# lior1990/hp-vae-gan

Measured on AMD Instinct MI355X. Metric: train iters/sec per pyramid scale, air_balloons 13f@144p, higher is better.
Workload: dtype f32

## Files before the change

hp-vae-gan_amd/csrc/conv_mfma.hip:

```cpp
#include "hpvg_common.h"
#include "hpvg.h"
#include <stdlib.h>

namespace {

__device__ const float g_zero_word[16] = {0.f, 0.f, 0.f, 0.f, 0.f, 0.f, 0.f, 0.f, 0.f, 0.f, 0.f, 0.f, 0.f, 0.f, 0.f, 0.f};
constexpr long HPVG_ZERO_PLANE_FLOATS = 1L << 18;
__device__ float g_zero_plane[HPVG_ZERO_PLANE_FLOATS];

#ifdef HPVG_TRACE
__device__ unsigned long long g_trace[8192 * 4];
__device__ unsigned long long g_phase[8192 * 4];
#define HPVG_PH(i) { unsigned long long now_ = __builtin_readcyclecounter(); ph_a[i] += now_ - ph_t; ph_t = now_; }
#define HPVG_PH_INIT unsigned long long ph_t = __builtin_readcyclecounter(); unsigned long long ph_a[4] = {0, 0, 0, 0};
#define HPVG_PH_END if (threadIdx.x == 0) { for (int i_ = 0; i_ < 4; ++i_) g_phase[4 * blockIdx.x + i_] = ph_a[i_]; }
#define HPVG_TRACE_BEGIN unsigned long long tr_t0 = wall_clock64(); unsigned long long tr_c0 = __builtin_readcyclecounter();
#define HPVG_TRACE_END                                                              \
  if (threadIdx.x == 0 && blockIdx.x + gridDim.x * (blockIdx.y + gridDim.y * blockIdx.z) < 8192) { \
    unsigned long long* tr = g_trace + 4 * (blockIdx.x + gridDim.x * (blockIdx.y + gridDim.y * blockIdx.z)); \
    tr[0] = tr_t0;                                                                  \
    tr[1] = wall_clock64();                                                         \
    tr[2] = __builtin_amdgcn_s_getreg((31 << 11) | 4);                              \
    tr[3] = (__builtin_amdgcn_s_getreg((31 << 11) | 20) & 0xF) | ((__builtin_readcyclecounter() - tr_c0) << 8); \
  }
// ... 161 lines not shown
#if HPVG_CONV_ASM_STAGE
        const unsigned dst_lds = (unsigned)(size_t)(lptr_t)dst;
#pragma unroll
        for (int j = 0; j < NJMAX; ++j)
          if (sl.em[j] != 0ull) conv_dma_piece(src, sl.bofs[j], dst_lds + j * 1024, sl.em[j]);
#else
#pragma unroll
        for (int j = 0; j < NJMAX; ++j)
          if ((sl.okmask >> j) & 1u)
            __builtin_amdgcn_global_load_lds((gptr_t)(src + sl.bofs[j]), (lptr_t)(dst + j * 256), 4, 0, 0);
#endif
        if (first_chunk) {
#pragma unroll
          for (int j = 0; j < NJMAX; ++j)
            if (((sl.wmask & ~sl.okmask) >> j) & 1u) xs[pl * PL + j * 256 + tid] = 0.f;
        }
      } else if (first_chunk || cg >= a.Cin) {
#pragma unroll
        for (int j = 0; j < NJMAX; ++j)
          if ((sl.wmask >> j) & 1u) xs[pl * PL + j * 256 + tid] = 0.f;
      }
    }
  } else {
#pragma unroll 2
    for (int c = 0; c < CC; ++c) {
      const int cg = ch * CC + c;
      const bool cok = cg < a.Cin;
      float sc = 1.f, sh = 0.f;
      if (cok) {
        sc = a.in_scale[cg];
        sh = a.in_shift[cg];
      }
      float v[KT][NJMAX];
#pragma unroll
      for (int dt = 0; dt < KT; ++dt) {
        const int tt = t + dt - (KT == 3 ? 1 : 0);
        const bool tok = cok && tt >= 0 && tt < a.T;
        const float* src = a.x + (((long)b * a.Cin + (cok ? cg : 0)) * a.T + (tok ? tt : 0)) * HW;
#pragma unroll
        for (int j = 0; j < NJMAX; ++j) {
          const bool ld = tok && ((sl.okmask >> j) & 1u);
          v[dt][j] = ld ? src[sl.gofs[j]] : 0.f;
        }
      }
#pragma unroll
      for (int dt = 0; dt < KT; ++dt) {
        const int tt = t + dt - (KT == 3 ? 1 : 0);
        const bool tok = cok && tt >= 0 && tt < a.T;
#pragma unroll
        for (int j = 0; j < NJMAX; ++j) {
          if ((sl.wmask >> j) & 1u) {
            float val = v[dt][j];
            if (tok && ((sl.okmask >> j) & 1u)) {
              val = val * sc + sh;
              if (a.in_lrelu) val = hpvg_lrelu(val);
            }
            xs[(c * KT + dt) * PL + j * 256 + tid] = val;
          }
        }
      }
    }
  }
}

#ifdef HPVG_CONV_WGS4
#define HPVG_CONV_WGS(MB, NB) ((MB) * (NB) <= 4 ? 4 : 2)
#else
#define HPVG_CONV_WGS(MB, NB) 2
#endif

constexpr int VAR_PLAIN = 0, VAR_MASK = 1, VAR_PRO = 2, VAR_BITS = 3;

template <int CC, int KT, int MB, int NB, int VAR>
__global__ __launch_bounds__(256, HPVG_CONV_WGS(MB, NB)) void conv_mfma_kernel(const ConvFwdArgs a) {
  constexpr int CP = CC / 2;
  constexpr int TAPS = KT * 9;
  typedef typename AVecT<CP>::type AVec;
  extern __shared__ __attribute__((aligned(16))) float xs[];

  const int tid = threadIdx.x;
  const int lane = tid & 63;
  const int wave = __builtin_amdgcn_readfirstlane(tid >> 6);
  const int half = lane >> 5, l31 = lane & 31;
  const long HW = (long)a.H * a.W;
  const int RS = a.RS, PL = a.PL;
  const float* xl = xs + half * KT * PL + l31 + wave * 32;

  HPVG_TRACE_BEGIN
  const int S = gridDim.x;
  const int g = hpvg_xcd_remap(blockIdx.x, S);
  const long Isk = (long)(a.ntl - a.skbase) * a.nchunk;
  int it = (int)((long)g * Isk / S);
  const int it_hi = (int)((long)(g + 1) * Isk / S);
  const int first_sk_tile = a.skbase + it / a.nchunk;

  HPVG_PH_INIT
  bool first_stage = true;
  for (int k = 0;; ++k) {
    int tile, ch_lo, ch_hi;
    if (k < a.ndp) {
      tile = k * S + g;
      ch_lo = 0;
      ch_hi = a.nchunk;
    } else {
      if (it >= it_hi) break;
      const int tr = it / a.nchunk;
      tile = a.skbase + tr;
      ch_lo = it - tr * a.nchunk;
      const int n = (a.nchunk - ch_lo < it_hi - it) ? a.nchunk - ch_lo : it_hi - it;
      ch_hi = ch_lo + n;
      it += n;
    }
    const SkTile tc = sk_decode_tile(a, tile, MB);
    const int b = tc.b, t = tc.t, q0 = tc.q0, w0 = tc.w0, mb0 = tc.mb0;

    const StageSlots sl = conv_stage_slots(a, q0, w0, tid);

    f32x16 acc[MB][NB];
#pragma unroll
    for (int m = 0; m < MB; ++m)
#pragma unroll
      for (int i = 0; i < NB; ++i)
#pragma unroll
        for (int e = 0; e < 16; ++e) acc[m][i][e] = 0.f;

    for (int ch = ch_lo; ch < ch_hi; ++ch) {
      if (!first_stage) __syncthreads();
      first_stage = false;
      HPVG_PH(3)
      __builtin_amdgcn_s_waitcnt(0x0F70);
      conv_stage_chunk<CC, KT, VAR == VAR_PRO>(a, xs, sl, ch, ch == ch_lo, b, t, tid, wave);
      HPVG_PH(0)
      __builtin_amdgcn_s_waitcnt(0x0F70);
      __syncthreads();
      HPVG_PH(1)

      const AVec* wpt = reinterpret_cast<const AVec*>(a.wp) + ((long)(ch * TAPS) * a.mbtot + mb0) * 64 + lane;
      AVec av[MB];
#pragma unroll
      for (int m = 0; m < MB; ++m) av[m] = wpt[m * 64];
      float bv[2][NB];
#pragma unroll
      for (int i = 0; i < NB; ++i) bv[0][i] = xl[i * 128];
#pragma unroll 1
      for (int dt = 0; dt < KT; ++dt) {
#pragma unroll
        for (int dh = 0; dh < 3; ++dh) {
#pragma unroll
          for (int dw = 0; dw < 3; ++dw) {
            wpt += (long)a.mbtot * 64;
            AVec an[MB];
#pragma unroll
            for (int m = 0; m < MB; ++m) an[m] = wpt[m * 64];
            const float* xt = xl + dt * PL + dh * RS + dw;
            const float* xn = (dw < 2) ? xt + 1 : (dh < 2 ? xl + dt * PL + (dh + 1) * RS : xl + (dt + 1 < KT ? dt + 1 : 0) * PL);
#pragma unroll
            for (int cp = 0; cp < CP; ++cp) {
              const float* nx = (cp + 1 < CP) ? xt + (2 * (cp + 1) * KT) * PL : xn;
#pragma unroll
              for (int i = 0; i < NB; ++i) bv[(cp + 1) & 1][i] = nx[i * 128];
              __builtin_amdgcn_sched_barrier(0);
              __builtin_amdgcn_s_setprio(1);
#pragma unroll
              for (int i = 0; i < NB; ++i)
#pragma unroll
                for (int m = 0; m < MB; ++m)
                  acc[m][i] = __builtin_amdgcn_mfma_f32_32x32x2f32(av[m][cp], bv[cp & 1][i], acc[m][i], 0, 0, 0);
              __builtin_amdgcn_s_setprio(0);
            }
#pragma unroll
            for (int m = 0; m < MB; ++m) av[m] = an[m];
          }
        }
      }
      HPVG_PH(2)
    }

    if (ch_lo != 0 || ch_hi != a.nchunk) {
      const int seg = (tile == first_sk_tile) ? 0 : 1;
      float* dst = a.skpart + ((long)(g * 2 + seg) * (MB * NB * 16)) * 256 + tid;
#pragma unroll
      for (int m = 0; m < MB; ++m)
#pragma unroll
        for (int i = 0; i < NB; ++i)
#pragma unroll
          for (int e = 0; e < 16; ++e) dst[((m * NB + i) * 16 + e) * 256] = acc[m][i][e];
      continue;
    }
    float bias_r[MB][16];
#pragma unroll
    for (int m = 0; m < MB; ++m)
#pragma unroll
      for (int e = 0; e < 16; ++e) {
        const int co = (mb0 + m) * 32 + (e & 3) + 8 * (e >> 2) + 4 * half;
        bias_r[m][e] = (a.bias && co < a.Cout) ? a.bias[co] : 0.f;
      }
#pragma unroll
    for (int i = 0; i < NB; ++i) {
      const int blk = wave + 4 * i;
      const int q = blk * 32 + l31;
      const int Q = q0 + q;
      const int gh = Q / RS, ww = Q - gh * RS;
      const int gw = w0 + ww;
      const bool ok = q < a.L && ww < a.Tw && gh < a.H && gw < a.W;
      const long sp = (long)t * HW + (long)gh * a.W + gw;
      const long wi = ((long)b * a.mbtot + mb0) * a.T * HW + sp;
      if constexpr (VAR == VAR_BITS) {
#pragma unroll
        for (int m = 0; m < MB; ++m) {
          unsigned word = 0;
#pragma unroll
          for (int e = 0; e < 16; ++e) {
            const float val = acc[m][i][e] + bias_r[m][e];
            word |= (val > 0.f ? 1u : 0u) << ((e & 3) + 8 * (e >> 2) + 4 * half);
          }
          word |= (unsigned)__shfl_xor((int)word, 32, 64);
          if (ok && half == 0 && (mb0 + m) * 32 < a.Cout) a.bits_out[wi + (long)m * a.T * HW] = word;
        }
      }
      if (!ok) continue;
      unsigned mword[MB];
      if constexpr (VAR == VAR_MASK) {
        if (a.mask_bits) {
#pragma unroll
          for (int m = 0; m < MB; ++m) mword[m] = (mb0 + m) * 32 < a.Cout ? a.mask_bits[wi + (long)m * a.T * HW] : 0u;
        }
      }
#pragma unroll
      for (int m = 0; m < MB; ++m) {
#pragma unroll
        for (int e = 0; e < 16; ++e) {
          const int co = (mb0 + m) * 32 + (e & 3) + 8 * (e >> 2) + 4 * half;
          if (co < a.Cout) {
            float val = acc[m][i][e] + bias_r[m][e];
            if (a.out_lrelu) val = hpvg_lrelu(val);
            const long oi = ((long)b * a.Cout + co) * a.T * HW + sp;
            if constexpr (VAR == VAR_MASK) {
              if (a.mask_bits) val *= ((mword[m] >> ((e & 3) + 8 * (e >> 2) + 4 * half)) & 1u) ? 1.f : HPVG_LRELU_SLOPE;
              else val *= a.mask[oi] > 0.f ? 1.f : HPVG_LRELU_SLOPE;
            }
            a.y[oi] = val;
          }
        }
      }
    }
  }
  HPVG_PH_END
  HPVG_TRACE_END
}

__global__ __launch_bounds__(256) void conv_fixup_kernel(const ConvFwdArgs a, int S, int MB, int NB) {
  const int r = blockIdx.x;
  const int mi = blockIdx.y;
  const int m = mi / NB, i = mi - m * NB;
  const long Isk = (long)(a.ntl - a.skbase) * a.nchunk;
  const long i0 = (long)r * a.nchunk, i1 = i0 + a.nchunk - 1;
  const int g0 = (int)(((i0 + 1) * S + Isk - 1) / Isk) - 1;
  const int g1 = (int)(((i1 + 1) * S + Isk - 1) / Isk) - 1;
  if (g0 == g1) return;
  const int tid = threadIdx.x;
  const int lane = tid & 63, wave = tid >> 6, half = lane >> 5, l31 = lane & 31;
  const SkTile tc = sk_decode_tile(a, a.skbase + r, MB);
  const long HW = (long)a.H * a.W;
  const int RS = a.RS;
  const int blk = wave + 4 * i;
  const int q = blk * 32 + l31;
  const int Q = tc.q0 + q;
  const int gh = Q / RS, ww = Q - gh * RS;
  const int gw = tc.w0 + ww;
  if (!(q < a.L && ww < a.Tw && gh < a.H && gw < a.W)) return;
  const long slab = (long)MB * NB * 16 * 256;
  float v[16];
#pragma unroll
  for (int e = 0; e < 16; ++e) v[e] = 0.f;
  for (int g = g0; g <= g1; ++g) {
    const long st = (long)g * Isk / S, en = (long)(g + 1) * Isk / S;
    if (st == en) continue;
    const int seg = (st / a.nchunk == r) ? 0 : 1;
    const float* src = a.skpart + (long)(g * 2 + seg) * slab + (long)mi * 16 * 256 + tid;
#pragma unroll
    for (int e = 0; e < 16; ++e) v[e] += src[e * 256];
  }
  const long sp = (long)tc.t * HW + (long)gh * a.W + gw;
  const long wi = ((long)tc.b * a.mbtot + tc.mb0 + m) * a.T * HW + sp;
  const unsigned mword = a.mask_bits ? a.mask_bits[wi] : 0u;
  unsigned word = 0;
#pragma unroll
  for (int e = 0; e < 16; ++e) {
    const int co = (tc.mb0 + m) * 32 + (e & 3) + 8 * (e >> 2) + 4 * half;
    if (co >= a.Cout) continue;
    float val = v[e];
    if (a.bias) val += a.bias[co];
    word |= (val > 0.f ? 1u : 0u) << ((e & 3) + 8 * (e >> 2) + 4 * half);
    if (a.out_lrelu) val = hpvg_lrelu(val);
    const long oi = ((long)tc.b * a.Cout + co) * a.T * HW + sp;
    if (a.mask_bits) val *= ((mword >> ((e & 3) + 8 * (e >> 2) + 4 * half)) & 1u) ? 1.f : HPVG_LRELU_SLOPE;
    else if (a.mask) val *= a.mask[oi] > 0.f ? 1.f : HPVG_LRELU_SLOPE;
    a.y[oi] = val;
  }
  if (a.bits_out) {
    word |= (unsigned)__shfl_xor((int)word, 32, 64);
    if (half == 0) a.bits_out[wi] = word;
  }
}

#include "conv_wino.inl"
#include "conv_wino2d.inl"
#include "conv_wino2r.inl"

template <int KT, int NT>
__global__ __launch_bounds__(256, 2) void conv_narrow_kernel(const ConvFwdArgs a, int ksteps, int pitch) {
  extern __shared__ __attribute__((aligned(16))) float P[];
  const int tid = threadIdx.x;
  const int lane = tid & 63;
  const int wave = __builtin_amdgcn_readfirstlane(tid >> 6);
  const int half = lane >> 5, l31 = lane & 31;
  const long HW = (long)a.H * a.W;
  const int RS = a.RS;
  const int CO9 = a.Cout * 9;
  const int pt = (KT == 3 ? 1 : 0);

  const int tile = hpvg_xcd_remap(blockIdx.x, gridDim.x);
  const SkTile tc = sk_decode_tile(a, tile, 1);
  const int b = tc.b, t = tc.t, h0 = tc.q0 / RS, w0 = tc.w0;
  const int plload = (a.Th + 2) * RS;
  const int nblk = (plload + 31) / 32;
  const float* xb0 = a.x + (long)b * a.Cin * a.T * HW;

  const int Kh = ksteps;
  for (int blk = wave; blk < nblk; blk += 4) {
    const int p = blk * 32 + l31;
    const int hh = p / RS, ww = p - hh * RS;
    const int gh = h0 + hh - 1, gw = w0 + ww - 1;
    const bool inimg = p < plload && gh >= 0 && gh < a.H && gw >= 0 && gw < a.W;
    const int kofs = half * Kh;
    const int c_h = kofs / KT, dt_h = kofs - c_h * KT;
    const unsigned lofs = (unsigned)((((long)c_h * a.T + dt_h) * HW + (inimg ? gh * a.W + gw : 0)) * 4);
    const char* xbase = reinterpret_cast<const char*>(a.x + ((long)b * a.Cin * a.T + (t - pt)) * HW);
    const float* wq = a.wp + lane;
    f32x16 acc[NT];
#pragma unroll
    for (int nt = 0; nt < NT; ++nt)
#pragma unroll
      for (int e = 0; e < 16; ++e) acc[nt][e] = 0.f;
    constexpr int KC = 16;
    float ab[2][KC], bb[2][NT][KC];
    auto load_chunk = [&](float (&av)[KC], float (&bv)[NT][KC], int s0) {
#pragma unroll
      for (int j = 0; j < KC; ++j) {
        const int s = s0 + j;
        const int cs = s / KT, ds = s - cs * KT;
        const int dtt = dt_h + ds;
        const int c = c_h + cs + (dtt >= KT ? 1 : 0);
        const int dt = dtt >= KT ? dtt - KT : dtt;
        const int tt = t + dt - pt;
        const bool ok = inimg && s < ksteps && c < a.Cin && tt >= 0 && tt < a.T;
        const long rel = (((long)(c - c_h) * a.T + (dt - dt_h)) * HW) * 4;
        float v = ok ? *reinterpret_cast<const float*>(xbase + rel + lofs) : 0.f;
        if (a.in_scale != nullptr && ok) {
          v = v * a.in_scale[c] + a.in_shift[c];
          if (a.in_lrelu) v = hpvg_lrelu(v);
        }
        av[j] = v;
#pragma unroll
        for (int nt = 0; nt < NT; ++nt) bv[nt][j] = s < ksteps ? wq[(s * NT + nt) * 64] : 0.f;
      }
    };
    auto mma_chunk = [&](const float (&av)[KC], const float (&bv)[NT][KC]) {
#pragma unroll
      for (int j = 0; j < KC; ++j)
#pragma unroll
        for (int nt = 0; nt < NT; ++nt) acc[nt] = __builtin_amdgcn_mfma_f32_32x32x2f32(av[j], bv[nt][j], acc[nt], 0, 0, 0);
    };
    load_chunk(ab[0], bb[0], 0);
    for (int s0 = 0; s0 < ksteps; s0 += 2 * KC) {
      load_chunk(ab[1], bb[1], s0 + KC);
      __builtin_amdgcn_sched_barrier(0);
      mma_chunk(ab[0], bb[0]);
      __builtin_amdgcn_sched_barrier(0);
      load_chunk(ab[0], bb[0], s0 + 2 * KC);
      __builtin_amdgcn_sched_barrier(0);
      mma_chunk(ab[1], bb[1]);
      __builtin_amdgcn_sched_barrier(0);
    }
#pragma unroll
    for (int nt = 0; nt < NT; ++nt) {
      const int n = nt * 32 + l31;
      if (n < CO9) {
#pragma unroll
        for (int e = 0; e < 16; ++e) P[n * pitch + blk * 32 + (e & 3) + 8 * (e >> 2) + 4 * half] = acc[nt][e];
      }
    }
  }
  __syncthreads();

  const int npos = a.Th * a.Tw;
  for (int idx = tid; idx < npos; idx += 256) {
    const int hh = idx / a.Tw, ww = idx - hh * a.Tw;
    const int gh = h0 + hh, gw = w0 + ww;
    if (gh >= a.H || gw >= a.W) continue;
    const long sp = (long)t * HW + (long)gh * a.W + gw;
    for (int o = 0; o < a.Cout; ++o) {
      float v = 0.f;
#pragma unroll
      for (int dh = 0; dh < 3; ++dh)
#pragma unroll
        for (int dw = 0; dw < 3; ++dw) v += P[(o * 9 + dh * 3 + dw) * pitch + (hh + dh) * RS + ww + dw];
      if (a.bias) v += a.bias[o];
      if (a.out_lrelu) v = hpvg_lrelu(v);
      const long oi = ((long)b * a.Cout + o) * a.T * HW + sp;
      if (a.mask) v *= a.mask[oi] > 0.f ? 1.f : HPVG_LRELU_SLOPE;
      a.y[oi] = v;
    }
  }
}


struct Narrow2Geom {
  int RS, Th, nth, nb, npos, G, pitch;
  int ws[16], ob[16], on[16];
};
typedef float f32x4u __attribute__((ext_vector_type(4), aligned(4)));
typedef float f32x2u __attribute__((ext_vector_type(2), aligned(4)));
template <int JB> struct AVecU;
template <> struct AVecU<4> { typedef f32x4u type; };
template <> struct AVecU<2> { typedef f32x2u type; };

template <int KT, int NT, int JB>
__global__ __launch_bounds__(256, 2) void conv_narrow2_kernel(const ConvFwdArgs a, const Narrow2Geom g, int ksteps) {
  typedef typename AVecU<JB>::type AV;
  constexpr int GP = 32 * JB;
  constexpr int KC = KT == 3 ? 6 : 8;
  extern __shared__ __attribute__((aligned(16))) float P[];
  const int tid = threadIdx.x;
  const int lane = tid & 63;
  const int wave = __builtin_amdgcn_readfirstlane(tid >> 6);
  const int half = lane >> 5, l31 = lane & 31;
  const long HW = (long)a.H * a.W;
  const int RS = g.RS, pitch = g.pitch;
  const int CO9 = a.Cout * 9;
  const int pt = (KT == 3 ? 1 : 0);

  int r = hpvg_xcd_remap(blockIdx.x, gridDim.x);
  const int band = r % g.nb; r /= g.nb;
  const int t = r % a.T; r /= a.T;
  const int th = r % g.nth;
  const int b = r / g.nth;
  const int h0 = th * g.Th, wsb = g.ws[band];
  const float* xs = a.x + ((long)b * a.Cin * a.T + (t - pt)) * HW;
  const int chalf = (ksteps / KT) * half;

  for (int grp = wave; grp < g.G; grp += 4) {
    const int p = GP * grp + JB * l31;
    const int pc = p < g.npos ? p : g.npos - JB;
    const int row = pc / RS, col = pc - row * RS;
    const int gh = h0 - 1 + row;
    const bool valid = p < g.npos && gh >= 0 && gh < a.H;
    const int ghc = gh < 0 ? 0 : (gh >= a.H ? a.H - 1 : gh);
    const float* lp = xs + (long)chalf * a.T * HW + (long)ghc * a.W + wsb + col;
    const float* wq = a.wp + lane;
    f32x16 acc[JB][NT];
#pragma unroll
    for (int j = 0; j < JB; ++j)
#pragma unroll
      for (int nt = 0; nt < NT; ++nt)
#pragma unroll
        for (int e = 0; e < 16; ++e) acc[j][nt][e] = 0.f;
    bool tok[KT];
#pragma unroll
    for (int dt = 0; dt < KT; ++dt) tok[dt] = (t + dt - pt >= 0) && (t + dt - pt < a.T);
    AV av[2][KC];
    float bv[2][KC][NT];
    auto load_chunk = [&](AV (&A)[KC], float (&Bf)[KC][NT], int s0) {
#pragma unroll
      for (int j = 0; j < KC; ++j) {
        const int s = s0 + j;
        const int dt = j % KT;
        const int cs = s0 / KT + j / KT;
        if (s < ksteps && tok[dt]) {
          A[j] = *reinterpret_cast<const AV*>(lp + ((long)cs * a.T + dt) * HW);
#pragma unroll
          for (int nt = 0; nt < NT; ++nt) Bf[j][nt] = wq[(s * NT + nt) * 64];
        }
      }
    };
    auto mma_chunk = [&](const AV (&A)[KC], const float (&Bf)[KC][NT], int s0) {
#pragma unroll
      for (int j = 0; j < KC; ++j) {
        const int s = s0 + j;
        if (s < ksteps && tok[j % KT]) {
#pragma unroll
          for (int jj = 0; jj < JB; ++jj) {
            const float v = valid ? A[j][jj] : 0.f;
#pragma unroll
            for (int nt = 0; nt < NT; ++nt) acc[jj][nt] = __builtin_amdgcn_mfma_f32_32x32x2f32(v, Bf[j][nt], acc[jj][nt], 0, 0, 0);
          }
        }
      }
    };
    load_chunk(av[0], bv[0], 0);
    for (int s0 = 0; s0 < ksteps; s0 += 2 * KC) {
      load_chunk(av[1], bv[1], s0 + KC);
      __builtin_amdgcn_sched_barrier(0);
      mma_chunk(av[0], bv[0], s0);
      __builtin_amdgcn_sched_barrier(0);
      load_chunk(av[0], bv[0], s0 + 2 * KC);
      __builtin_amdgcn_sched_barrier(0);
      mma_chunk(av[1], bv[1], s0 + KC);
      __builtin_amdgcn_sched_barrier(0);
    }
#pragma unroll
    for (int nt = 0; nt < NT; ++nt) {
      const int n = nt * 32 + l31;
      if (n < CO9) {
#pragma unroll
        for (int jj = 0; jj < JB; ++jj)
#pragma unroll
          for (int e = 0; e < 16; ++e) P[n * pitch + GP * grp + JB * ((e & 3) + 8 * (e >> 2) + 4 * half) + jj] = acc[jj][nt][e];
      }
    }
  }
  __syncthreads();

  const int ob = g.ob[band], on = g.on[band];
  const int nout = g.Th * on;
  for (int idx = tid; idx < nout; idx += 256) {
    const int hh = idx / on, cc = idx - hh * on;
    const int gh = h0 + hh, gw = ob + cc;
    if (gh >= a.H) continue;
    const long sp = (long)t * HW + (long)gh * a.W + gw;
    for (int o = 0; o < a.Cout; ++o) {
      float v = 0.f;
#pragma unroll
      for (int dh = 0; dh < 3; ++dh)
#pragma unroll
        for (int dw = 0; dw < 3; ++dw) {
          const int gwt = gw + dw - 1;
          if (gwt >= 0 && gwt < a.W) v += P[(o * 9 + dh * 3 + dw) * pitch + (hh + dh) * RS + (gwt - wsb)];
        }
      if (a.bias) v += a.bias[o];
      if (a.out_lrelu) v = hpvg_lrelu(v);
      a.y[((long)b * a.Cout + o) * a.T * HW + sp] = v;
    }
  }
}

bool plan_narrow2(int B, int Cin, int Cout, int T, int H, int W, int KT, Narrow2Geom* out, long* ntiles) {
  if ((Cin & 1) || W < 4) return false;
  const int NT = hpvg_cdiv(9 * Cout, 32);
  const int JB = NT == 1 ? 4 : 2;
  const int GP = 32 * JB;
  double best = 1e300;
  bool found = false;
  auto bands = [&](int RS, Narrow2Geom* q) -> int {
    int nb = 0, o = 0;
    while (o < W) {
      if (nb == 16) return 0;
      int n, ws;
      if (nb == 0) { n = (RS == W) ? W : RS - 1; ws = 0; }
      else if (W - o <= RS - 1) { n = W - o; ws = W - RS; }
      else { n = RS - 2; ws = o - 1; }
      if (n < 1) return 0;
      if (q) { q->ws[nb] = ws; q->ob[nb] = o; q->on[nb] = n; }
      o += n;
      ++nb;
    }
    return nb;
  };
  for (int RS = 4; RS <= 256 && RS <= W; RS += 4) {
    const int nb = bands(RS, nullptr);
    if (nb == 0) continue;
    for (int Th = 1; Th <= H; ++Th) {
      const int nth = hpvg_cdiv(H, Th);
      if (Th != hpvg_cdiv(H, nth)) continue;
      const int npos = (Th + 2) * RS;
      const int G = hpvg_cdiv(npos, GP);
      if (G > 16) break;
      const int pitch = (G * GP) | 1;
      if ((size_t)(9 * Cout) * pitch * sizeof(float) > 76 * 1024) break;
      const long nt = (long)B * T * nth * nb;
      const double rounds = hpvg_cdiv(G, 4);
      const double waves = nt <= 2L * HPVG_NUM_CU ? 1.0 : (double)nt / (2.0 * HPVG_NUM_CU);
      const double cost = waves * (rounds * GP + 30.0);
      if (cost < best) {
        best = cost;
        found = true;
        Narrow2Geom q{};
        q.RS = RS; q.Th = Th; q.nth = nth; q.nb = nb; q.npos = npos; q.G = G; q.pitch = pitch;
        bands(RS, &q);
        *out = q;
        *ntiles = nt;
      }
    }
  }
  if (!found) return false;
  for (int k = 0; k < out->nb; ++k) {
    const int lo = out->ob[k] - 1 < 0 ? 0 : out->ob[k] - 1;
    const int hi = out->ob[k] + out->on[k] > W - 1 ? W - 1 : out->ob[k] + out->on[k];
    if (out->on[k] < 0 || lo < out->ws[k] || hi >= out->ws[k] + out->RS) return false;
  }
  return true;
}

template <int KT>
int launch_conv_narrow2(const ConvFwdArgs& a, const Narrow2Geom& g, long ntiles, hipStream_t s) {
  const int ksteps = hpvg_cdiv(a.Cin * KT, 2);
// ... 318 lines not shown

static const bool g_wino2r = [] { const char* e = getenv("HPVG_WINO2R"); return !e || atoi(e) != 0; }();
int g_wino2d = 0;
struct W2Geom { int Cq, R, ntq, tqw, gridy, nsc, ntl; bool ok; };
inline W2Geom wino2d_geom(int B, int Cin, int Cout, int T, int H, int W, int KT) {
  W2Geom q{};
  if (!conv_is_wino2d(Cin, Cout, KT) || ((W & 1) && !g_wino2r) || W < 2 || (long)H * W < 4) return q;
  if (g_wino2r && (long)H * W + 4 > HPVG_ZERO_PLANE_FLOATS) return q;
  q.Cq = (W + 1) / 2;
  q.R = hpvg_cdiv(H, 2);
  const int nq = q.R * q.Cq;
  q.ntq = hpvg_cdiv(nq, 64);
  q.tqw = 64;
  for (int tp = 0; tp < q.ntq; ++tp) {
    const int Q0 = tp * 64, R0 = Q0 / q.Cq, c0 = Q0 - R0 * q.Cq;
    int Ql = Q0 + 63;
    if (Ql > nq - 1) Ql = nq - 1;
    const int R1 = Ql / q.Cq, c1 = Ql - R1 * q.Cq;
    const int lo = (2 * R0 - 1) * W + 2 * c0 - 1;
    const int lo4 = lo >= 0 ? (lo & ~3) : -((3 - lo) & ~3);
    const int hi = (2 * R1 + 2) * W + 2 * c1 + 3;
    if (hi - lo4 > 1024) return q;
  }
  q.gridy = hpvg_cdiv(hpvg_cdiv(Cout, 32), 2);
  q.nsc = hpvg_cdiv(Cin, 4);
  const long ntl = (long)B * T * q.ntq * q.gridy;
  if (ntl > 0x7fffffffL) return q;
  q.ntl = (int)ntl;
  q.ok = true;
  return q;
}
inline bool conv_use_wino2d(const W2Geom& q, bool prologue) {
  if (!q.ok || prologue || g_wino2d == 1 || g_wino_mode == 0) return false;
  if (g_wino2d == 2) return true;
  const long rounds = (q.ntl + HPVG_NUM_CU - 1) / HPVG_NUM_CU;
  if (rounds == 1) return q.ntl * 2 >= HPVG_NUM_CU;
  return (long)q.ntl * 10 >= 6L * rounds * HPVG_NUM_CU;
}
template <typename K>
int launch_wino2d_kern(K kern, bool& attr_set, const Wino2Args& a, hipStream_t s) {
  if (!attr_set) {
    if (hipFuncSetAttribute(reinterpret_cast<const void*>(kern), hipFuncAttributeMaxDynamicSharedMemorySize, 160 * 1024) != hipSuccess)
      (void)hipGetLastError();
    attr_set = true;
  }
  const int S = a.ntl < HPVG_NUM_CU ? a.ntl : HPVG_NUM_CU;
  hipLaunchKernelGGL(kern, dim3(S), dim3(256), (size_t)3 * 12 * W2_PL * sizeof(float), s, a);
  return hpvg_launch_status();
}
template <int VAR, bool TAIL>
int launch_wino2d_inst(const Wino2Args& a, hipStream_t s) {
  static bool attr_r = false, attr_o = false, attr_d = false;
  if (a.W & 1) return launch_wino2d_kern(conv_wino2r_kernel<VAR, TAIL, true>, attr_o, a, s);
  if (g_wino2r) return launch_wino2d_kern(conv_wino2r_kernel<VAR, TAIL, false>, attr_r, a, s);
  return launch_wino2d_kern(conv_wino2d_kernel<VAR, TAIL>, attr_d, a, s);
}

template <int VAR>
int launch_wino2d_var(const Wino2Args& a, hipStream_t s) {
  return (((long)a.H * a.W) & 3) ? launch_wino2d_inst<VAR, true>(a, s) : launch_wino2d_inst<VAR, false>(a, s);
}

inline bool conv_is_narrow(int Cin, int Cout) { return Cout <= 4 && Cin > 4; }

Plan plan_conv(int B, int Cin, int Cout, int T, int H, int W, int KT, bool streamk, bool wino = false) {
  const bool narrow = conv_is_narrow(Cin, Cout);
  if (narrow) streamk = false;
  struct Key { int B, Cin, Cout, T, H, W, KT, sk; };
  struct Entry { Key k; Plan p; bool used; };
  constexpr int NSLOT = 2048;
  static thread_local Entry cache[NSLOT];
  static thread_local int filled = 0;
  const Key k{B, Cin, Cout, T, H, W, KT, (streamk ? 1 : 0) | (wino ? 2 : 0) | (wino ? g_wino_stg << 2 : 0)};
  unsigned h = 2166136261u;
  for (int v : {B, Cin, Cout, T, H, W, KT, k.sk}) h = (h ^ (unsigned)v) * 16777619u;
  for (int probe = 0; probe < NSLOT; ++probe) {
    Entry& e = cache[(h + probe) & (NSLOT - 1)];
    if (!e.used) {
      const Plan p = wino ? plan_wino_search(B, Cin, Cout, T, H, W, KT, streamk) : plan_conv_search(B, Cin, Cout, T, H, W, KT, streamk, narrow);
      if (filled < NSLOT / 2) {
        e.k = k; e.p = p; e.used = true;
        ++filled;
      }
      return p;
    }
    const Key& c = e.k;
    if (c.B == B && c.Cin == Cin && c.Cout == Cout && c.T == T && c.H == H && c.W == W && c.KT == KT && c.sk == k.sk) return e.p;
  }
  return wino ? plan_wino_search(B, Cin, Cout, T, H, W, KT, streamk) : plan_conv_search(B, Cin, Cout, T, H, W, KT, streamk, narrow);
}

constexpr size_t CONV_MIN_LDS = 56 * 1024;
template <int CC, int KT, int MB, int NB, int VAR>
int launch_conv_var(const ConvFwdArgs& a, const Plan& p, int S, hipStream_t s) {
  static bool attr_set = false;
  auto kern = conv_mfma_kernel<CC, KT, MB, NB, VAR>;
  if (!attr_set) {
    if (hipFuncSetAttribute(reinterpret_cast<const void*>(kern), hipFuncAttributeMaxDynamicSharedMemorySize, 160 * 1024) !=
        hipSuccess)
      (void)hipGetLastError();
    attr_set = true;
  }
  const size_t min_lds = HPVG_CONV_WGS(MB, NB) == 4 ? (size_t)33 * 1024 : CONV_MIN_LDS;
  hipLaunchKernelGGL(kern, dim3(S), dim3(256), p.lds < min_lds ? min_lds : p.lds, s, a);
  int rc = hpvg_launch_status();
  if (rc != HPVG_OK) return rc;
  const int nsk = a.ntl - a.skbase;
  if (nsk > 0) {
    hipLaunchKernelGGL(conv_fixup_kernel, dim3(nsk, MB * NB), dim3(256), 0, s, a, S, MB, NB);
    rc = hpvg_launch_status();
  }
  return rc;
}

template <int CC, int KT, int MB, int NB>
int launch_conv(const ConvFwdArgs& a, const Plan& p, int S, hipStream_t s) {
  if (a.in_scale) return launch_conv_var<CC, KT, MB, NB, VAR_PRO>(a, p, S, s);
  if (a.mask || a.mask_bits) return launch_conv_var<CC, KT, MB, NB, VAR_MASK>(a, p, S, s);
  if (a.bits_out) return launch_conv_var<CC, KT, MB, NB, VAR_BITS>(a, p, S, s);
  return launch_conv_var<CC, KT, MB, NB, VAR_PLAIN>(a, p, S, s);
}

template <int CC, int KT>
int dispatch_conv(const ConvFwdArgs& a, const Plan& p, int S, hipStream_t s) {
  if (p.MB == 2) {
    switch (p.NB) {
      case 1: return launch_conv<CC, KT, 2, 1>(a, p, S, s);
      case 2: return launch_conv<CC, KT, 2, 2>(a, p, S, s);
      default: return launch_conv<CC, KT, 2, 4>(a, p, S, s);
    }
  }
  switch (p.NB) {
    case 1: return launch_conv<CC, KT, 1, 1>(a, p, S, s);
    case 2: return launch_conv<CC, KT, 1, 2>(a, p, S, s);
    default: return launch_conv<CC, KT, 1, 4>(a, p, S, s);
  }
}

template <int KT, int VAR, int STG>
int launch_wino_var(const ConvFwdArgs& a, const Plan& p, int S, hipStream_t s) {
  static bool attr_set = false;
  auto kern = conv_wino_kernel<KT, WINO_NBP, VAR, STG>;
  if (!attr_set) {
    if (hipFuncSetAttribute(reinterpret_cast<const void*>(kern), hipFuncAttributeMaxDynamicSharedMemorySize, 160 * 1024) !=
        hipSuccess)
      (void)hipGetLastError();
    attr_set = true;
  }
  hipLaunchKernelGGL(kern, dim3(S), dim3(256), p.lds < CONV_MIN_LDS ? CONV_MIN_LDS : p.lds, s, a);
  int rc = hpvg_launch_status();
  if (rc != HPVG_OK) return rc;
  const int nsk = a.ntl - a.skbase;
  if (nsk > 0) {
    hipLaunchKernelGGL(conv_wino_fixup_kernel, dim3(nsk, WINO_NBP * 2), dim3(256), 0, s, a, S, WINO_NBP);
    rc = hpvg_launch_status();
  }
  return rc;
}

template <int KT, int STG>
int launch_wino_stg(const ConvFwdArgs& a, const Plan& p, int S, hipStream_t s) {
  if (a.mask || a.mask_bits) return launch_wino_var<KT, VAR_MASK, STG>(a, p, S, s);
  if (a.bits_out) return launch_wino_var<KT, VAR_BITS, STG>(a, p, S, s);
  return launch_wino_var<KT, VAR_PLAIN, STG>(a, p, S, s);
}
template <int KT>
int launch_wino(const ConvFwdArgs& a, const Plan& p, int S, hipStream_t s) {
  return p.stg == 2 ? launch_wino_stg<KT, 2>(a, p, S, s) : launch_wino_stg<KT, 1>(a, p, S, s);
}

template <int KT>
int launch_conv_narrow(const ConvFwdArgs& a, const Plan& p, hipStream_t s) {
  const int ksteps = hpvg_cdiv(a.Cin * KT, 2);
  const int pitch = (hpvg_cdiv((p.Th + 2) * p.RS, 32) * 32) | 1;
  const size_t lds = (size_t)(9 * a.Cout) * pitch * sizeof(float);
#define HPVG_NARROW(NT)                                                                                              \
  {                                                                                                                  \
    static bool attr = false;                                                                                        \
    if (!attr) {                                                                                                     \
      if (hipFuncSetAttribute(reinterpret_cast<const void*>(conv_narrow_kernel<KT, NT>),                             \
                              hipFuncAttributeMaxDynamicSharedMemorySize, 160 * 1024) != hipSuccess)                 \
        (void)hipGetLastError();                                                                                     \
      attr = true;                                                                                                   \
    }                                                                                                                \
    hipLaunchKernelGGL((conv_narrow_kernel<KT, NT>), dim3(a.ntl), dim3(256), lds, s, a, ksteps, pitch);              \
  }
  if (9 * a.Cout <= 32) HPVG_NARROW(1) else HPVG_NARROW(2)
#undef HPVG_NARROW
  return hpvg_launch_status();
}

inline int conv_sk_grid(int ntl, int nchunk, const Plan& p) {
  const long items = (long)ntl * nchunk;
  const long slots = conv_slots(p.MB, p.NB);
  return (int)(items < slots ? items : slots);
}
inline size_t conv_sk_ws_bytes(const Plan& p, int S) { return (size_t)S * 2 * p.MB * p.NB * 16 * 256 * sizeof(float); }

}

extern "C" {

static size_t wpack_floats_impl(int Cin, int Cout, int KT, bool with2d) {
  if (conv_is_narrow(Cin, Cout)) return (size_t)hpvg_cdiv(Cin * KT, 2) * hpvg_cdiv(9 * Cout, 32) * 64;
  return direct_pack_floats(Cin, Cout, KT) + (conv_is_wino(Cin, Cout) ? wino_pack_floats(Cin, Cout, KT) : 0) +
         (with2d && conv_is_wino2d(Cin, Cout, KT) ? wino2_pack_floats(Cin, Cout) : 0);
}
static bool wants_wino2d(int B, int Cin, int Cout, int T, int H, int W, int KT) {
  if (B < 1 || T < 1 || H < 1 || W < 1 || !conv_use_wino(B, Cin, Cout, T, H, W, KT, false)) return false;
  return conv_use_wino2d(wino2d_geom(B, Cin, Cout, T, H, W, KT), false);
}
size_t hpvg_conv_wpack_floats(int Cin, int Cout, int KT) { return wpack_floats_impl(Cin, Cout, KT, true); }
size_t hpvg_conv_wpack_floats_for(int Cin, int Cout, int KT, int B, int T, int H, int W) {
  return wpack_floats_impl(Cin, Cout, KT, wants_wino2d(B, Cin, Cout, T, H, W, KT));
}
int hpvg_conv_wants_wino2d(int B, int Cin, int Cout, int T, int H, int W, int KT) { return wants_wino2d(B, Cin, Cout, T, H, W, KT) ? 1 : 0; }

static int pack_weight_impl(const float* w, const float* inv_scale, float* wp, int Cin_layer, int Cout_layer, int KT,
                            int transpose_flip, bool with2d, void* stream);
int hpvg_conv_pack_weight_f32(const float* w, const float* inv_scale, float* wp, int Cin_layer, int Cout_layer, int KT,
                              int transpose_flip, void* stream) {
  return pack_weight_impl(w, inv_scale, wp, Cin_layer, Cout_layer, KT, transpose_flip, true, stream);
}
int hpvg_conv_pack_weight_for_f32(const float* w, const float* inv_scale, float* wp, int Cin_layer, int Cout_layer, int KT,
                                  int transpose_flip, int B, int T, int H, int W, void* stream) {
  const int Cin_k = transpose_flip ? Cout_layer : Cin_layer, Cout_k = transpose_flip ? Cin_layer : Cout_layer;
  return pack_weight_impl(w, inv_scale, wp, Cin_layer, Cout_layer, KT, transpose_flip, wants_wino2d(B, Cin_k, Cout_k, T, H, W, KT), stream);
}
static int pack_weight_impl(const float* w, const float* inv_scale, float* wp, int Cin_layer, int Cout_layer, int KT,
                            int transpose_flip, bool with2d, void* stream) {
  if (!w || !wp || (KT != 1 && KT != 3) || Cin_layer < 1 || Cout_layer < 1) return HPVG_ERR_ARG;
  const int Cin_k = transpose_flip ? Cout_layer : Cin_layer;
  const int Cout_k = transpose_flip ? Cin_layer : Cout_layer;
  if (conv_is_narrow(Cin_k, Cout_k)) {
    const long total = (long)wpack_floats_impl(Cin_k, Cout_k, KT, with2d);
    hipLaunchKernelGGL(conv_pack_narrow_kernel, dim3(hpvg_cdiv(total, 256)), dim3(256), 0, (hipStream_t)stream, w, inv_scale, wp,
                       Cin_k, Cout_k, KT, hpvg_cdiv(9 * Cout_k, 32), hpvg_cdiv(Cin_k * KT, 2), transpose_flip, total);
    return hpvg_launch_status();
  }
  const int CC = conv_cc(Cin_k);
  const int nchunk = hpvg_cdiv(Cin_k, CC);
  const int mbtot = hpvg_cdiv(Cout_k, 32);
  const long total = (long)wpack_floats_impl(Cin_k, Cout_k, KT, with2d);
  hipLaunchKernelGGL(conv_pack_kernel, dim3(hpvg_cdiv(total, 256)), dim3(256), 0, (hipStream_t)stream, w, inv_scale, wp,
                     Cin_k, Cout_k, KT * 9, CC, nchunk, mbtot, transpose_flip, (long)direct_pack_floats(Cin_k, Cout_k, KT), total);
  return hpvg_launch_status();
}

static int pack_batch_impl(int n, const float* const* w, float* const* wp, const int* flip, int C, int KT, bool with2d, void* stream);
int hpvg_conv_pack_weight_batch_f32(int n, const float* const* w, float* const* wp, const int* flip, int C, int KT, void* stream) {
  return pack_batch_impl(n, w, wp, flip, C, KT, true, stream);
}
int hpvg_conv_pack_weight_batch_for_f32(int n, const float* const* w, float* const* wp, const int* flip, int C, int KT, int B, int T,
                                        int H, int W, void* stream) {
  return pack_batch_impl(n, w, wp, flip, C, KT, wants_wino2d(B, C, C, T, H, W, KT), stream);
}
static int pack_batch_impl(int n, const float* const* w, float* const* wp, const int* flip, int C, int KT, bool with2d, void* stream) {
  if (n < 1 || n > HPVG_PACK_BATCH_MAX || !w || !wp || !flip || C <= 4 || (KT != 1 && KT != 3)) return HPVG_ERR_ARG;
  PackBatchArgs a;
  for (int i = 0; i < n; ++i) {
    if (!w[i] || !wp[i]) return HPVG_ERR_ARG;
    a.w[i] = w[i]; a.wp[i] = wp[i]; a.flip[i] = flip[i];
  }
  const int CC = conv_cc(C);
  const int nchunk = hpvg_cdiv(C, CC);
  const int mbtot = hpvg_cdiv(C, 32);
  const long total = (long)wpack_floats_impl(C, C, KT, with2d);
  hipLaunchKernelGGL(conv_pack_batch_kernel, dim3(hpvg_cdiv(total, 256), n), dim3(256), 0, (hipStream_t)stream, a, C, KT * 9, CC,
                     nchunk, mbtot, (long)direct_pack_floats(C, C, KT), total);
  return hpvg_launch_status();
}

static int conv_fwd_impl(const float* x, const float* wp, const float* bias, const float* in_scale, const float* in_shift,
                         int in_lrelu, float* y, int out_lrelu, const float* out_mask, const unsigned* mask_bits, unsigned* bits_out,
                         void* ws, size_t ws_bytes, int B, int Cin, int Cout, int T, int H, int W, int KT, void* stream);

int hpvg_conv_fwd_f32(const float* x, const float* wp, const float* bias, const float* in_scale, const float* in_shift,
                      int in_lrelu, float* y, int out_lrelu, const float* out_mask, void* ws, size_t ws_bytes, int B, int Cin,
                      int Cout, int T, int H, int W, int KT, void* stream) {
  return conv_fwd_impl(x, wp, bias, in_scale, in_shift, in_lrelu, y, out_lrelu, out_mask, nullptr, nullptr, ws, ws_bytes, B, Cin,
                       Cout, T, H, W, KT, stream);
}

size_t hpvg_conv_mask_words(int B, int C, int T, int H, int W) { return (size_t)B * T * H * W * hpvg_cdiv(C, 32); }

int hpvg_conv_fwd_bits_f32(const float* x, const float* wp, const float* bias, float* y, int out_lrelu, const unsigned* mask_bits,
                           unsigned* bits_out, void* ws, size_t ws_bytes, int B, int Cin, int Cout, int T, int H, int W, int KT,
                           void* stream) {
  if (conv_is_narrow(Cin, Cout)) return HPVG_ERR_UNSUPPORTED;
  if (mask_bits && bits_out) return HPVG_ERR_UNSUPPORTED;
  return conv_fwd_impl(x, wp, bias, nullptr, nullptr, 0, y, out_lrelu, nullptr, mask_bits, bits_out, ws, ws_bytes, B, Cin, Cout, T, H,
                       W, KT, stream);
}

static int conv_fwd_impl(const float* x, const float* wp, const float* bias, const float* in_scale, const float* in_shift,
                         int in_lrelu, float* y, int out_lrelu, const float* out_mask, const unsigned* mask_bits, unsigned* bits_out,
                         void* ws, size_t ws_bytes, int B, int Cin, int Cout, int T, int H, int W, int KT, void* stream) {
  if (!x || !wp || !y) return HPVG_ERR_ARG;
  if (B < 1 || Cin < 1 || Cout < 1 || T < 1 || H < 1 || W < 1) return HPVG_ERR_ARG;
  if (KT != 1 && KT != 3) return HPVG_ERR_UNSUPPORTED;
  if ((in_scale == nullptr) != (in_shift == nullptr)) return HPVG_ERR_ARG;
  if (in_scale && out_mask && !conv_is_narrow(Cin, Cout)) return HPVG_ERR_UNSUPPORTED;
  static const bool sk_off = [] { const char* e = getenv("HPVG_CONV_SK"); return e && atoi(e) == 0; }();
  const int CC = conv_cc(Cin);
  const int nchunk = hpvg_cdiv(Cin, CC);
  bool streamk = !sk_off && ws != nullptr && !conv_is_narrow(Cin, Cout);
  bool wino = conv_use_wino(B, Cin, Cout, T, H, W, KT, in_scale != nullptr);
  if (wino) {
    const W2Geom q2 = wino2d_geom(B, Cin, Cout, T, H, W, KT);
    if (conv_use_wino2d(q2, in_scale != nullptr) && !out_mask) {
      Wino2Args w2;
      w2.x = x; w2.bias = bias; w2.mask_bits = mask_bits; w2.bits_out = bits_out; w2.y = y;
      w2.wp = wp + direct_pack_floats(Cin, Cout, KT) + wino_pack_floats(Cin, Cout, KT);
      w2.B = B; w2.Cin = Cin; w2.Cout = Cout; w2.T = T; w2.H = H; w2.W = W;
      w2.Cq = q2.Cq; w2.R = q2.R; w2.ntq = q2.ntq; w2.tqw = q2.tqw; w2.mbtot = wino2_mb(Cout); w2.gridy = q2.gridy;
      w2.nsc = q2.nsc; w2.ntl = q2.ntl; w2.PL = W2_PL; w2.out_lrelu = out_lrelu; w2.mbreal = hpvg_cdiv(Cout, 32);
      Wino2Args a2 = w2;
      hipStream_t s2 = (hipStream_t)stream;
      if (mask_bits) return launch_wino2d_var<VAR_MASK>(a2, s2);
      if (bits_out) return launch_wino2d_var<VAR_BITS>(a2, s2);
      return launch_wino2d_var<VAR_PLAIN>(a2, s2);
    }
  }
  Plan p = plan_conv(B, Cin, Cout, T, H, W, KT, streamk, wino);
  if (wino && p.L == 0) {
    wino = false;
    p = plan_conv(B, Cin, Cout, T, H, W, KT, streamk, false);
  }
  if (p.L == 0) return HPVG_ERR_UNSUPPORTED;
  int ntl = B * T * p.nrange * p.ntw * p.gridy;
  if (streamk && ws_bytes < conv_sk_ws_bytes(p, conv_sk_grid(ntl, nchunk, p))) {
    streamk = false;
    p = plan_conv(B, Cin, Cout, T, H, W, KT, false, wino);
    if (p.L == 0) return HPVG_ERR_UNSUPPORTED;
    ntl = B * T * p.nrange * p.ntw * p.gridy;
  }
  ConvFwdArgs a;
  a.x = x; a.wp = wp; a.bias = bias; a.in_scale = in_scale; a.in_shift = in_shift; a.mask = out_mask; a.y = y;
  a.mask_bits = mask_bits; a.bits_out = bits_out;
  a.B = B; a.Cin = Cin; a.Cout = Cout; a.T = T; a.H = H; a.W = W;
  a.Th = p.Th; a.Tw = p.Tw; a.RS = p.RS; a.PL = p.PL; a.L = p.L; a.qstride = p.qstride; a.nrange = p.nrange; a.ntw = p.ntw; a.nblocks = p.nblocks;
  a.nchunk = nchunk;
  a.mbtot = hpvg_cdiv(Cout, 32);
  a.nj = p.nj;
  a.in_lrelu = in_lrelu; a.out_lrelu = out_lrelu;
  a.gridy = p.gridy;
  a.ntl = ntl;
  if (conv_is_narrow(Cin, Cout)) {
    a.ndp = 1; a.skbase = ntl; a.skpart = nullptr;
    static const bool n2_off = [] { const char* e = getenv("HPVG_NARROW2"); return e && atoi(e) == 0; }();
    Narrow2Geom g2;
    long nt2 = 0;
    if (!n2_off && !in_scale && !out_mask && plan_narrow2(B, Cin, Cout, T, H, W, KT, &g2, &nt2))
      return KT == 3 ? launch_conv_narrow2<3>(a, g2, nt2, (hipStream_t)stream) : launch_conv_narrow2<1>(a, g2, nt2, (hipStream_t)stream);
    return KT == 3 ? launch_conv_narrow<3>(a, p, (hipStream_t)stream) : launch_conv_narrow<1>(a, p, (hipStream_t)stream);
  }
  const int S = streamk ? conv_sk_grid(ntl, nchunk, p) : ntl;
  a.ndp = ntl / S;
  a.skbase = a.ndp * S;
  a.skpart = (float*)ws;
  hipStream_t s = (hipStream_t)stream;
  a.stagger = 0;
  if (wino) {
    static const int stagger_env = [] { const char* e = getenv("HPVG_WINO_STAGGER"); return e ? atoi(e) : 0; }();
    a.stagger = (S > HPVG_NUM_CU) ? stagger_env : 0;
    a.wp = wp + direct_pack_floats(Cin, Cout, KT);
    return KT == 3 ? launch_wino<3>(a, p, S, s) : launch_wino<1>(a, p, S, s);
  }
  if (CC == 8) return KT == 3 ? dispatch_conv<8, 3>(a, p, S, s) : dispatch_conv<8, 1>(a, p, S, s);
  return KT == 3 ? dispatch_conv<4, 3>(a, p, S, s) : dispatch_conv<4, 1>(a, p, S, s);
}

int hpvg_conv_fwd_kernel_kind(int B, int Cin, int Cout, int T, int H, int W, int KT) {
  if (B < 1 || Cin < 1 || Cout < 1 || T < 1 || H < 1 || W < 1 || (KT != 1 && KT != 3)) return HPVG_ERR_ARG;
  if (conv_is_narrow(Cin, Cout)) return 3;
  if (!conv_use_wino(B, Cin, Cout, T, H, W, KT, false)) return 0;
  if (conv_use_wino2d(wino2d_geom(B, Cin, Cout, T, H, W, KT), false)) return 2;
  return plan_conv(B, Cin, Cout, T, H, W, KT, true, true).L != 0 ? 1 : 0;
}

size_t hpvg_conv_fwd_ws_bytes(int B, int Cin, int Cout, int T, int H, int W, int KT) {
  if (B < 1 || Cin < 1 || Cout < 1 || T < 1 || H < 1 || W < 1 || (KT != 1 && KT != 3)) return 0;
  if (conv_is_narrow(Cin, Cout)) return 0;
  size_t need = 0;
  for (int wino = 0; wino < 2; ++wino) {
    if (wino && !conv_use_wino(B, Cin, Cout, T, H, W, KT, false)) break;
    const Plan p = plan_conv(B, Cin, Cout, T, H, W, KT, true, wino != 0);
    if (p.L == 0) continue;
    const size_t n = conv_sk_ws_bytes(p, conv_sk_grid(B * T * p.nrange * p.ntw * p.gridy, hpvg_cdiv(Cin, conv_cc(Cin)), p));
    if (n > need) need = n;
  }
  return need;
}

int hpvg_conv_fwd_plan(int B, int Cin, int Cout, int T, int H, int W, int KT, int* out) {
  if (!out || (KT != 1 && KT != 3)) return HPVG_ERR_ARG;
  const Plan p = plan_conv(B, Cin, Cout, T, H, W, KT, true);
  out[0] = p.L; out[1] = p.Tw; out[2] = p.nrange; out[3] = p.ntw; out[4] = p.nblocks; out[5] = p.NB; out[6] = p.MB;
  out[7] = p.gridy; out[8] = (int)p.lds; out[9] = B * T * p.nrange * p.ntw;
  return HPVG_OK;
}

int hpvg_conv_wino_config(int mode, long min_positions) {
  if (wino_env_mode() == 0) return HPVG_ERR_UNSUPPORTED;
  (void)conv_use_wino(1, 8, 64, 1, 1, 1, 3, false);
  if (mode >= 0) {
    g_wino_mode = mode > 2 ? 2 : mode;
    g_wino_stg = mode == 3 ? 2 : (mode == 4 ? 1 : 0);
    g_wino2d = mode == 5 ? 2 : (mode == 3 || mode == 4 || mode == 6 ? 1 : 0);
  }
  if (min_positions >= 0) g_wino_min_pos = min_positions;
  if (g_wino_mode == 2 && g_wino2d == 2) return 5;
  if (g_wino_mode == 2 && g_wino_stg) return g_wino_stg == 2 ? 3 : 4;
  if (g_wino_mode == 2 && g_wino2d == 1) return 6;
  return g_wino_mode;
}

int hpvg_conv_wino_plan(int B, int Cin, int Cout, int T, int H, int W, int KT, int* out) {
  if (!out || (KT != 1 && KT != 3) || B < 1 || Cin < 1 || Cout < 1 || T < 1 || H < 1 || W < 1) return HPVG_ERR_ARG;
  if (!conv_is_wino(Cin, Cout)) return HPVG_ERR_UNSUPPORTED;
  const Plan p = plan_conv(B, Cin, Cout, T, H, W, KT, true, true);
  if (p.L == 0) return HPVG_ERR_UNSUPPORTED;
  out[0] = p.L; out[1] = p.Tw; out[2] = p.nrange; out[3] = p.ntw; out[4] = p.RS; out[5] = p.NB; out[6] = p.MB;
  out[7] = p.gridy; out[8] = (int)p.lds; out[9] = B * T * p.nrange * p.ntw * p.gridy;
  return HPVG_OK;
}

int hpvg_conv_narrow_plan(int B, int Cin, int Cout, int T, int H, int W, int KT, int* out) {
  if (!out || (KT != 1 && KT != 3)) return HPVG_ERR_ARG;
  Narrow2Geom g;
  long nt = 0;
  if (!conv_is_narrow(Cin, Cout) || !plan_narrow2(B, Cin, Cout, T, H, W, KT, &g, &nt)) return HPVG_ERR_UNSUPPORTED;
  out[0] = g.RS; out[1] = g.Th; out[2] = g.nth; out[3] = g.nb; out[4] = g.npos; out[5] = g.G; out[6] = g.pitch;
  for (int k = 0; k < g.nb; ++k) { out[7 + 3 * k] = g.ws[k]; out[8 + 3 * k] = g.ob[k]; out[9 + 3 * k] = g.on[k]; }
  return HPVG_OK;
}

#ifdef HPVG_TRACE
int hpvg_debug_phase_read(unsigned long long* host_out, int n) {
  return hipMemcpyFromSymbol(host_out, HIP_SYMBOL(g_phase), sizeof(unsigned long long) * 4 * n) == hipSuccess ? 0 : -4;
}
int hpvg_debug_trace_read(unsigned long long* host_out, int n) {
  return hipMemcpyFromSymbol(host_out, HIP_SYMBOL(g_trace), sizeof(unsigned long long) * 4 * n) == hipSuccess ? 0 : -4;
}
#endif

}
```

Measured before the change: 31.72.

## Add direct FMA conv kernel for tiny-Cin inputs instead of MFMA path

Adds a specialized forward conv kernel for layers with at most four input channels. Each thread computes one output pixel for 32 output channels using scalar FMAs over a 3x3xKT stencil, reading packed MFMA weights directly. It is dispatched ahead of the MFMA/Winograd paths when the spatial size is large enough. The aim is to avoid wasting MFMA K-dimension padding and tiling overhead on the RGB input layer. The trade-off is more scalar arithmetic and uncached redundant neighbour loads from global memory.

```diff
diff --git a/hp-vae-gan_amd/csrc/conv_mfma.hip b/hp-vae-gan_amd/csrc/conv_mfma.hip
--- a/hp-vae-gan_amd/csrc/conv_mfma.hip
+++ b/hp-vae-gan_amd/csrc/conv_mfma.hip
@@ -487,6 +487,119 @@
     word |= (unsigned)__shfl_xor((int)word, 32, 64);
     if (half == 0) a.bits_out[wi] = word;
   }
+}
+
+template <int KT, int CIN>
+__global__ __launch_bounds__(256) void conv_narrow_in_kernel(const ConvFwdArgs a, const float* __restrict__ wp) {
+  constexpr int pt = KT == 3 ? 1 : 0;
+  constexpr int G = CIN == 1 ? 16 : 8;
+  const int HW = a.H * a.W;
+  const int t = blockIdx.y % a.T, b = blockIdx.y / a.T;
+  const int p = blockIdx.x * 256 + threadIdx.x;
+  if (blockIdx.x * 256 + (threadIdx.x & ~63) >= HW) return;
+  const bool live = p < HW;
+  const int pc = live ? p : HW - 1;
+  const int h = pc / a.W, w = pc - h * a.W;
+  const bool hok[3] = {h > 0, true, h + 1 < a.H};
+  const bool wok[3] = {w > 0, true, w + 1 < a.W};
+  const int mb = blockIdx.z;
+  const bool pro = a.in_scale != nullptr;
+
+  float acc[32];
+#pragma unroll
+  for (int i = 0; i < 32; ++i) acc[i] = 0.f;
+
+  typedef float f32x16u __attribute__((ext_vector_type(16), aligned(4)));
+#pragma unroll
+  for (int dt = 0; dt < KT; ++dt) {
+    const int tt = t + dt - pt;
+    if (tt < 0 || tt >= a.T) continue;
+    float v[CIN][9];
+#pragma unroll
+    for (int c = 0; c < CIN; ++c) {
+      const float* xp = a.x + ((long)(b * CIN + c) * a.T + tt) * HW + pc;
+      const float sc = pro ? a.in_scale[c] : 1.f, sh = pro ? a.in_shift[c] : 0.f;
+#pragma unroll
+      for (int dh = 0; dh < 3; ++dh)
+#pragma unroll
+        for (int dw = 0; dw < 3; ++dw) {
+          float u = 0.f;
+          if (hok[dh] && wok[dw]) {
+            u = xp[(dh - 1) * a.W + (dw - 1)];
+            if (pro) {
+              u = u * sc + sh;
+              if (a.in_lrelu) u = hpvg_lrelu(u);
+            }
+          }
+          v[c][dh * 3 + dw] = u;
+        }
+    }
+#pragma unroll
+    for (int k = 0; k < 9; ++k) {
+      const float* wt = wp + ((long)(dt * 9 + k) * a.mbtot + mb) * 128;
+#pragma unroll
+      for (int q = 0; q < 32 / G; ++q) {
+        if constexpr (CIN == 1) {
+          const f32x16u wa = *reinterpret_cast<const f32x16u*>(wt + q * 32);
+          const f32x16u wb = *reinterpret_cast<const f32x16u*>(wt + q * 32 + 16);
+#pragma unroll
+          for (int j = 0; j < 8; ++j) acc[q * 16 + j] = fmaf(wa[2 * j], v[0][k], acc[q * 16 + j]);
+#pragma unroll
+          for (int j = 0; j < 8; ++j) acc[q * 16 + 8 + j] = fmaf(wb[2 * j], v[0][k], acc[q * 16 + 8 + j]);
+        } else {
+          const f32x16u wa = *reinterpret_cast<const f32x16u*>(wt + q * 16);
+          const f32x16u wb = *reinterpret_cast<const f32x16u*>(wt + 64 + q * 16);
+#pragma unroll
+          for (int j = 0; j < 8; ++j) {
+            float s = fmaf(wa[2 * j], v[0][k], acc[q * 8 + j]);
+            s = fmaf(wb[2 * j], v[1][k], s);
+            if constexpr (CIN > 2) s = fmaf(wa[2 * j + 1], v[2][k], s);
+            if constexpr (CIN > 3) s = fmaf(wb[2 * j + 1], v[3][k], s);
+            acc[q * 8 + j] = s;
+          }
+        }
+        __builtin_amdgcn_sched_barrier(0);
+      }
+    }
+  }
+  if (!live) return;
+
+  const long THW = (long)a.T * HW;
+  const long sp = (long)t * HW + p;
+  const long wi = ((long)b * a.mbtot + mb) * THW + sp;
+  const unsigned mword = a.mask_bits ? a.mask_bits[wi] : 0u;
+  unsigned word = 0;
+#pragma unroll
+  for (int i = 0; i < 32; ++i) {
+    const int co = mb * 32 + i;
+    if (co < a.Cout) {
+      float val = acc[i];
+      if (a.bias) val += a.bias[co];
+      word |= (val > 0.f ? 1u : 0u) << i;
+      if (a.out_lrelu) val = hpvg_lrelu(val);
+      const long oi = ((long)b * a.Cout + co) * THW + sp;
+      if (a.mask_bits) val *= ((mword >> i) & 1u) ? 1.f : HPVG_LRELU_SLOPE;
+      else if (a.mask) val *= a.mask[oi] > 0.f ? 1.f : HPVG_LRELU_SLOPE;
+      a.y[oi] = val;
+    }
+  }
+  if (a.bits_out) a.bits_out[wi] = word;
+}
+
+inline bool conv_use_narrow_in(int B, int Cin, int T, int H, int W) {
+  return Cin <= 4 && (long)B * T * H * W >= (Cin == 1 ? 32768L : 200000L) && (long)H * W <= 0x7FFFFFFFL - 256 && (long)B * T <= 65535;
+}
+
+template <int KT>
+int launch_conv_narrow_in(const ConvFwdArgs& a, hipStream_t s) {
+  const dim3 grid((unsigned)hpvg_cdiv((long)a.H * a.W, 256), (unsigned)(a.B * a.T), (unsigned)a.mbtot);
+  switch (a.Cin) {
+    case 1: hipLaunchKernelGGL((conv_narrow_in_kernel<KT, 1>), grid, dim3(256), 0, s, a, a.wp); break;
+    case 2: hipLaunchKernelGGL((conv_narrow_in_kernel<KT, 2>), grid, dim3(256), 0, s, a, a.wp); break;
+    case 3: hipLaunchKernelGGL((conv_narrow_in_kernel<KT, 3>), grid, dim3(256), 0, s, a, a.wp); break;
+    default: hipLaunchKernelGGL((conv_narrow_in_kernel<KT, 4>), grid, dim3(256), 0, s, a, a.wp); break;
+  }
+  return hpvg_launch_status();
 }
 
 #include "conv_wino.inl"
@@ -1411,6 +1524,15 @@
   if ((in_scale == nullptr) != (in_shift == nullptr)) return HPVG_ERR_ARG;
   if (in_scale && out_mask && !conv_is_narrow(Cin, Cout)) return HPVG_ERR_UNSUPPORTED;
   static const bool sk_off = [] { const char* e = getenv("HPVG_CONV_SK"); return e && atoi(e) == 0; }();
+  if (conv_use_narrow_in(B, Cin, T, H, W)) {
+    ConvFwdArgs a{};
+    a.x = x; a.wp = wp; a.bias = bias; a.in_scale = in_scale; a.in_shift = in_shift; a.mask = out_mask; a.y = y;
+    a.mask_bits = mask_bits; a.bits_out = bits_out;
+    a.B = B; a.Cin = Cin; a.Cout = Cout; a.T = T; a.H = H; a.W = W;
+    a.mbtot = hpvg_cdiv(Cout, 32);
+    a.in_lrelu = in_lrelu; a.out_lrelu = out_lrelu;
+    return KT == 3 ? launch_conv_narrow_in<3>(a, (hipStream_t)stream) : launch_conv_narrow_in<1>(a, (hipStream_t)stream);
+  }
   const int CC = conv_cc(Cin);
   const int nchunk = hpvg_cdiv(Cin, CC);
   bool streamk = !sk_off && ws != nullptr && !conv_is_narrow(Cin, Cout);
```

After: 31.99 (median of 6 runs). About the same (+0.8%).
